# daihangpku/SW-NeRF

Measured on AMD Instinct MI355X. Metric: rays/sec (64+128 samples/ray), higher is better.
Workload: dtype f32

## Files before the change

### __graft_entry__.py

```python
import os
import subprocess
import sys

ROOT = os.path.dirname(os.path.abspath(__file__))
PKG = os.path.join(ROOT, "sw-nerf_amd")
CSRC = os.path.join(PKG, "csrc")
LIB = os.path.join(PKG, "swnerf", "libswnerf_hip.so")
SOURCES = ["render_kernels.hip", "train_kernels.hip", "misc_kernels.hip", "pack_kernels.hip", "backward_kernels.hip", "wgrad_kernels.hip", "wgrad_x3_kernels.hip", "generic_kernels.hip", "x3_kernels.hip", "mesh_kernels.hip", "tnerf_kernels.hip", "tnerf_train_kernels.hip", "metrics_kernels.hip", "pyramid_kernels.hip", "fit2d_kernels.hip", "batch_kernels.hip", "optim_kernels.hip", "patch_kernels.hip", "query_kernels.hip", "image_kernels.hip", "lpips_kernels.hip", "jpeg_kernels.hip", "jpeg_enc_kernels.hip", "marker_kernels.hip", "meshops_kernels.hip", "meshsimp_kernels.hip", "meshfill_kernels.hip"]
HEADERS = ["swnerf_common.h", "mlp_core.h", "mlp_core_x3.h", "bf16x3_split.h", "mlp_kernels.h", "render_pass.h", "composite.h", "resample.h", "wave_dpp.h", "lds_dma.h", "host_util.h", "wgrad_host.h", "mc_tables.h", "elu.h", "ray_rows.h", "tnerf_pass.h", "pyramid_interp.h", "jpeg_math.h", "jpeg_host.h", "jpeg_enc_math.h", "jpeg_enc_host.h", "marker_math.h", "meshops_math.h", "meshops_layout.h", "meshops_common.h", "par_prims.h", "fit2d_cols.h", os.path.join(ROOT, "include", "swnerf.h")]
HIPCC_FLAGS = ["--offload-arch=gfx950", "-O3", "-ffp-contract=off", "-fPIC", "-shared", "-std=c++17"]


OBJDIR = os.path.join(PKG, "build")


def _deps():
    return [os.path.join(CSRC, s) for s in SOURCES] + [h if os.path.isabs(h) else os.path.join(CSRC, h) for h in HEADERS]


def _stale():
    if not os.path.exists(LIB):
        return True
    t = os.path.getmtime(LIB)
    return any(os.path.getmtime(d) > t for d in _deps())


def compile_library(force=False):
    if not (force or _stale()):
        return False
    from concurrent.futures import ThreadPoolExecutor
    hipcc = os.environ.get("HIPCC", "/opt/rocm/bin/hipcc")
# ... 110 lines not shown
```

### include/swnerf.h

```cpp
#ifndef SWNERF_H
#define SWNERF_H
#include <stddef.h>
#include <stdint.h>

#ifdef __cplusplus
extern "C" {
#endif

#define SWNERF_VERSION 112

#define SWNERF_E_ARG      (-1)
#define SWNERF_E_UNSUPP   (-2)
#define SWNERF_E_DATA     (-3)

#define SWNERF_NET_CANON   0
#define SWNERF_NET_DNERF   1
#define SWNERF_NET_NOVIEW  2
#define SWNERF_NET_TNERF   3


int         swnerf_version(void);
const char* swnerf_last_error(void);

size_t swnerf_packed_floats(int kind);
// ... 102 lines not shown
    const float* z_vals;
    int          lindisp;
    const float* t_rand;
    const float* noise;
    int          white_bkgd;
    float* rgb_map;
    float* disp_map;
    float* acc_map;
    float* depth_map;
    float* weights;
    float* raw;
    float* dx;
    float* z_out;
    int          n_importance;
    const float* u;
    float* z_fine;
    float* z_std;
    int          out_ch;
} swnerf_pass_args;

int swnerf_render_pass(const swnerf_pass_args* args , void* stream);

int swnerf_render_pass_ws(const swnerf_pass_args* args , float* view_ws, int64_t view_ws_floats, void* stream);

size_t swnerf_packed_x3_floats_kind(int kind);
int swnerf_pack_net_x3_kind(int kind, const float* const* params , int L_pos, int L_dir, int L_time,
                            const float* packed_fp32, float* packed_x3, void* stream);
size_t swnerf_packed_x3_floats(void);
int swnerf_pack_net_x3(const float* const* params , int L_pos, int L_dir, const float* packed_canon,
                       float* packed_x3, void* stream);
int swnerf_render_pass_x3(const swnerf_pass_args* args , int terms, void* stream);

int64_t swnerf_train_rows(int64_t n_rays, int n_samples);
int swnerf_xs_floats_per_row(void);
int swnerf_render_pass_train(const swnerf_pass_args* args , float* act, float* bits, float* xs, void* stream);
int swnerf_render_pass_backward(const float* packed_bwd, const float* bits, const float* raw ,
                                const float* z_vals , const float* ray_batch, int cols, const float* noise,
                                int64_t n_rays, int n_samples, int white_bkgd, const float* g_rgb ,
                                const float* g_disp , const float* g_acc , const float* g_raw ,
                                float* grad, float* d_raw, void* stream);
size_t swnerf_packed_bwd_noview_floats(void);
int swnerf_pack_net_bwd_noview(const float* const* params , int L_pos, int out_ch,
                               float* packed_bwd, void* stream);
int swnerf_render_pass_backward_noview(const float* packed_bwd, const float* bits, const float* raw ,
                                       const float* z_vals , const float* ray_batch, int cols, const float* noise,
                                       int64_t n_rays, int n_samples, int white_bkgd, int out_ch, const float* g_rgb ,
// ... 210 lines not shown
```

### sw-nerf_amd/csrc/composite.h

```cpp
#pragma once
#include "wave_dpp.h"

typedef float f32x4 __attribute__((ext_vector_type(4)));

__device__ __forceinline__ float comp_dist(bool more, float zn, float z, float dnorm) {
    return (more ? (zn - z) : 1e10f) * dnorm;
}

__device__ __forceinline__ float comp_relu(float sg) { return (sg < 0.f) ? 0.f : sg; }

__device__ __forceinline__ float comp_transmit(float sg, float dist) { return expf(-comp_relu(sg) * dist); }

__device__ __forceinline__ float comp_alpha(float sg, float dist, bool live) {
    return live ? 1.f - comp_transmit(sg, dist) : 0.f;
}

__device__ __forceinline__ double comp_survival(float alpha) { return (double)(1.f - alpha + 1e-10f); }

struct SweepProd { double ex, total; };

template <int W>
__device__ __forceinline__ SweepProd excl_cumprod_shfl(double ps, int l) {
#pragma unroll
    for (int o = 1; o < W; o <<= 1) { const double up = __shfl_up(ps, o, W); if (l >= o) ps *= up; }
// ... 14 lines not shown

__device__ __forceinline__ float comp_sigmoid(float x) { return 1.f / (1.f + expf(-x)); }

__device__ __forceinline__ void comp_accumulate(const float& w, const float& c0, const float& c1, const float& c2, const float& z,
                                                float& pr, float& pg, float& pb, float& pd, float& pa) {
    pr += w * comp_sigmoid(c0);
    pg += w * comp_sigmoid(c1);
    pb += w * comp_sigmoid(c2);
    pd += w * z;
    pa += w;
}

__device__ __forceinline__ void comp_accumulate_density(const float& w, const float& z, float& pd, float& pa) {
    pd += w * z;
    pa += w;
}
__device__ __forceinline__ void comp_accumulate_colour(const float& w, const float& c0, const float& c1, const float& c2,
                                                       float& pr, float& pg, float& pb) {
    pr += w * comp_sigmoid(c0);
    pg += w * comp_sigmoid(c1);
    pb += w * comp_sigmoid(c2);
}

__device__ __forceinline__ void comp_write_maps(float pr, float pg, float pb, float pd, float pa, int white, int64_t ray,
                                                float* rgb_map, float* disp_map, float* acc_map, float* depth_map) {
    if (rgb_map) {
        const float bg = white ? (1.f - pa) : 0.f;
        rgb_map[ray * 3 + 0] = pr + bg;
        rgb_map[ray * 3 + 1] = pg + bg;
        rgb_map[ray * 3 + 2] = pb + bg;
    }
    if (depth_map) depth_map[ray] = pd;
    if (acc_map) acc_map[ray] = pa;
    if (disp_map) {
        const float q = pd / pa;
        disp_map[ray] = 1.f / ((q != q) ? q : fmaxf(1e-10f, q));
    }
}

struct CompGrads { float r, g, b, A, D; bool rgb; };

__device__ __forceinline__ void comp_bwd_fold(CompGrads& g, int white, const float* g_disp, float pd, float pa) {
    if (white) g.A -= (g.r + g.g + g.b);
    if (g_disp) {
        const float q = pd / pa;
        if (q > 1e-10f) { const float gq = -*g_disp / (q * q); g.D += gq / pa; g.A -= gq * pd / (pa * pa); }
    }
}

__device__ __forceinline__ float comp_bwd_G(const CompGrads& g, float c0, float c1, float c2, float z) {
    return (g.rgb ? g.r * c0 + g.g * c1 + g.b * c2 : 0.f) + g.A + g.D * z;
}

__device__ __forceinline__ f32x4 comp_bwd_sample(const CompGrads& g, float G, float T, float w, double R, float sg, float dist,
// ... 9 lines not shown
```

### sw-nerf_amd/csrc/render_kernels.hip

```cpp
#include <hip/hip_runtime.h>
#include "../../include/swnerf.h"
#include "swnerf_common.h"
#include "mlp_core.h"
#include "host_util.h"
#include "mlp_kernels.h"

#include "render_pass.h"

struct QueryDev {
    const float* pts; int64_t M; const float* dirs; int64_t V; int shared;
    const float* w0; const float* b0; int nbias; const float* wvl; float* out;
};

__global__ void __launch_bounds__(256, 1) query_points_kernel(QueryDev P) {
    extern __shared__ __attribute__((aligned(16))) float lds_bias[];
    RowTile rt;
    if (!row_tile(rt, lds_bias, P.b0, P.nbias, P.M)) return;
    f32x16 emb[2], in[8], out[8];
    float head[3];
    pe_pos(P.pts[rt.rr * 3], P.pts[rt.rr * 3 + 1], P.pts[rt.rr * 3 + 2], rt.h, emb);
    WStream ws;
    ws_start(ws, P.w0 + SW_STEPS_DIR * SW_STEP_FLOATS, lds_bias + SW_DIR_BIAS_TILES * SW_BIAS_TILE_FLOATS, rt.lds_ring, rt.lane);
    trunk_pass<false>(emb, rt.lds_emb, 0.f, false, rt.h, in, out, head, ws);
    float rgb[3];
    views_mean(in, ws, P.wvl, P.dirs, P.V, P.shared, rt.rr, rt.h, lds_bias, rgb);
    if (rt.live && rt.h == 0) {
        f32x4 r4 = {rgb[0], rgb[1], rgb[2], head[0]};
        *reinterpret_cast<f32x4*>(P.out + rt.row * 4) = r4;
    }
}

int sw_tnerf_render_launch(const swnerf_pass_args& a, hipStream_t st);

extern "C" int swnerf_render_pass_ws(const swnerf_pass_args* args, float* view_ws, int64_t view_ws_floats, void* stream) {
    static const PassAccepts accepts = {"render_pass", {SW_COLS(11) | SW_COLS(12), SW_COLS(11) | SW_COLS(12), SW_COLS(8), ~0u },
        SWNERF_E_ARG, "%s: ray_batch must have 11 or 12 columns (use_viewdirs) or 8 (SWNERF_NET_NOVIEW), got %d for kind %d", true, 0};
    if (!args) return sw_fail(SWNERF_E_ARG, "render_pass: NULL args");
    const swnerf_pass_args& a = *args;
    if (a.kind < 0 || a.kind > SWNERF_NET_TNERF) return sw_fail(SWNERF_E_ARG, "unknown net kind %d", a.kind);
    int rc = pass_check(accepts, a);
    if (rc) return rc;
    if (a.kind == SWNERF_NET_TNERF) return sw_tnerf_render_launch(a, (hipStream_t)stream);
    const bool noview = a.kind == SWNERF_NET_NOVIEW;
    if (a.kind == SWNERF_NET_DNERF && a.cols != 12) return sw_fail(SWNERF_E_ARG, "render_pass: D-NeRF needs the frame_time column");
    if (noview && a.dx) return sw_fail(SWNERF_E_ARG, "render_pass: a static net has no position_delta output here");
    PassDev P = pass_dev(a);
    rc = noview ? stream_ptrs_noview(a.packed, a.out_ch, &P.w0, &P.b0, &P.nbias, &P.two_pass)
                : stream_ptrs(a.kind, a.packed, a.run_deform, &P.w0, &P.b0, &P.nbias, &P.two_pass);
    if (rc) return rc;
    P.dir_steps = noview ? 0 : SW_STEPS_DIR;
    P.time_steps = (a.kind == SWNERF_NET_DNERF && P.two_pass) ? SW_STEPS_TIME : 0;
    size_t lds = SW_LDS_FIXED_FLOATS * sizeof(float);
    if ((rc = pass_resampling(accepts.name, a, P, lds))) return rc;
    if (view_ws && view_ws_floats < a.n_rays * (int64_t)SW_DEFER_WS_FLOATS)
        return sw_fail(SWNERF_E_ARG, "render_pass: view_ws holds %lld floats, %lld rays need %lld", (long long)view_ws_floats,
                       (long long)a.n_rays, (long long)(a.n_rays * (int64_t)SW_DEFER_WS_FLOATS));
    P.view_ws = (a.kind == SWNERF_NET_CANON && !a.raw && a.n_samples <= SW_DEFER_SMAX) ? view_ws : nullptr;
    if (P.view_ws && a.n_importance <= 0) lds += 4 * SW_DEFER_LDS_FLOATS * sizeof(float);
    if (a.n_rays == 0) return 0;
    if (P.time_steps) {
        P.tb_off = (int)(lds / sizeof(float));
        lds += 4 * SW_TB_LDS_FLOATS * sizeof(float);
    }
    const dim3 grid((unsigned)((a.n_rays + 3) / 4)), block(256);
    hipStream_t st = (hipStream_t)stream;
    pass_startup_args(P, grid.x, noview ? SW_NOVIEW_STEPS : (a.kind == SWNERF_NET_DNERF && P.two_pass ? SW_DEFORM_STEPS + SW_CANON_STEPS : SW_CANON_STEPS));
    if (noview) hipLaunchKernelGGL((render_pass_kernel<false, false, 0, false>), grid, block, lds, st, P);
    else if (a.kind == SWNERF_NET_DNERF) hipLaunchKernelGGL(render_pass_kernel<true>, grid, block, lds, st, P);
    else {
        if (a.dx) {
            rc = sw_check(hipMemsetAsync(a.dx, 0, (size_t)a.n_rays * a.n_samples * 3 * sizeof(float), st), "render_pass dx fill");
            if (rc) return rc;
        }
        hipLaunchKernelGGL(render_pass_kernel<false>, grid, block, lds, st, P);
    }
    return sw_check(hipGetLastError(), "render_pass launch");
}

extern "C" int swnerf_render_pass(const swnerf_pass_args* args, void* stream) { return swnerf_render_pass_ws(args, nullptr, 0, stream); }

__global__ void __launch_bounds__(256) sample_coarse_kernel(swnerf_pass_args a, float* z_out, float* pts) {
    const int64_t idx = (int64_t)blockIdx.x * 256 + threadIdx.x;
    const int S = a.n_samples;
    if (idx >= a.n_rays * S) return;
    const int64_t ray = idx / S;
    const int s = (int)(idx - ray * S);
    const float* rb = a.ray_batch + ray * a.cols;
    const float z = z_sample(a, ray, rb[6], rb[7], s);
    z_out[idx] = z;
    if (pts) {
        pts[idx * 3 + 0] = rb[0] + rb[3] * z;
        pts[idx * 3 + 1] = rb[1] + rb[4] * z;
        pts[idx * 3 + 2] = rb[2] + rb[5] * z;
    }
}

extern "C" int swnerf_sample_coarse(const float* ray_batch, int64_t n_rays, int cols, int n_samples, int lindisp,
                                    const float* t_rand, float* z_vals, float* pts, void* stream) {
    if (n_rays == 0) return 0;
    if (!ray_batch || !z_vals || n_rays < 0 || n_samples < 1 || cols < 8)
        return sw_fail(SWNERF_E_ARG, "sample_coarse: NULL pointer, n_rays %lld, n_samples %d or cols %d < 8", (long long)n_rays, n_samples, cols);
    swnerf_pass_args a = {};
// ... 72 lines not shown
```

### sw-nerf_amd/csrc/render_pass.h

```cpp
#pragma once
#include <cstdlib>
#include "mlp_kernels.h"
#include "mlp_core_x3.h"
#include "resample.h"
#include "composite.h"
#include "ray_rows.h"

#define SW_LDS_SC 256
#define SW_LDS_SORT 1024
#define SW_LDS_WAVE_FLOATS (3 * SW_LDS_SC + SW_LDS_SORT)

#define SW_DEFER_SMAX 240
#define SW_DEFER_LDS_FLOATS (4 * SW_DEFER_SMAX + 64)
#define SW_DEFER_WS_FLOATS (64 * 256)
static_assert(SW_DEFER_LDS_FLOATS <= SW_LDS_SORT, "the deferred colour scratch shares the sort region");

struct PassDev {
    swnerf_pass_args a;
    const float* w0;
    const float* b0;
    int nbias;
    int two_pass;
    int sort_n, sort_s;
    float* act;
    float* bits;
    float* xs;
    float* act_d; float* bits_d; float* xs_d;
    int dir_steps;
    int time_steps;
    int tb_off;
    int warm_steps;
    int warm_blocks;
    int skew_mode;
    int skew_unit;
    float* view_ws;
};

__device__ __forceinline__ float wave32_sum(float v) {
#pragma unroll
    for (int o = 16; o > 0; o >>= 1) v += __shfl_xor(v, o, 32);
    return v;
}

__device__ __forceinline__ float z_linear(const swnerf_pass_args& a, float near, float far, int s) {
    const float t = sw_linspace(0.f, 1.f, a.n_samples, s);
    if (!a.lindisp) return near * (1.f - t) + far * t;
    return 1.f / (1.f / near * (1.f - t) + 1.f / far * t);
}

__device__ __forceinline__ float z_sample(const swnerf_pass_args& a, int64_t ray, float near, float far, int s) {
    const int S = a.n_samples;
    if (a.z_vals) return a.z_vals[ray * S + s];
    const float zs = z_linear(a, near, far, s);
    if (!a.t_rand) return zs;
    const float upper = (s < S - 1) ? .5f * (z_linear(a, near, far, s + 1) + zs) : zs;
    const float lower = (s > 0) ? .5f * (zs + z_linear(a, near, far, s - 1)) : zs;
    return lower + (upper - lower) * a.t_rand[ray * S + s];
}
// ... 185 lines not shown
            tile_park(lds_dir, lane, demb);
        }
        x3_start(xs, reinterpret_cast<const char*>(P.w0), lds_bias, lds_ring, lane, wv);
    } else {
        ws_start(ws, P.w0, lds_bias, lds_ring, lane);
        if constexpr (VIEWS) {
            f32x16 demb;
            pe_dir(v0, v1, v2, h, demb);
            if constexpr (TRAIN) tile_park(lds_dir, lane, demb);
            view_bias_tile(demb, lds_vb, lane, ws);
        }
        if constexpr (DNERF) {
            if (P.time_steps) time_bias_tile(ft, h, lds_all + P.tb_off + wv * SW_TB_LDS_FLOATS, lane, ws);
        }
    }

    const float* zrow = a.z_vals ? a.z_vals + ray * S : nullptr;
    const float* zslot = PREC ? lds_x3w + X3Lds<DNERF>::DIR : lds_emb + SW_EMB_LDS_FLOATS;
    const unsigned zslot_addr = __builtin_amdgcn_readfirstlane((unsigned)(size_t)zslot);
    float pr = 0.f, pg = 0.f, pb = 0.f, pd = 0.f, pa = 0.f;
    double Tc = 1.0;
    const int ntiles = (S + 31) >> 5;
    constexpr bool DEFER_OK = !DNERF && !TRAIN && PREC == 0 && VIEWS;
    const bool defer = DEFER_OK && P.view_ws != nullptr;
    float* dW = resample ? srt : lds_all + PassLds<DNERF, TRAIN>::FIXED + wv * SW_DEFER_LDS_FLOATS;
    float* dC = dW + SW_DEFER_SMAX;
    int* dIdx = reinterpret_cast<int*>(dW + 4 * SW_DEFER_SMAX);
    float* vrow = DEFER_OK ? P.view_ws + ray * SW_DEFER_WS_FLOATS + h * 128 : nullptr;
    const char* main_head = reinterpret_cast<const char*>(P.w0 + (P.dir_steps + P.time_steps) * SW_STEP_FLOATS);
    const char* viewsh_head = main_head + (SW_CANON_MAIN_STEPS - SW_STEPS_VIEWSH) * 1024;
    int pend = 0, wr = 0, rd = 0;
    if constexpr (DEFER_OK) {
        if (defer) {
            for (int i = lane; i < 3 * SW_DEFER_SMAX; i += 64) dC[i] = 0.f;
            wave_lds_sync();
        }
    }
#pragma nounroll
    for (int tile = 0; tile < ntiles || (DEFER_OK && pend > 0); ++tile) {
        const bool is_tile = !DEFER_OK || tile < ntiles;
        const bool flush = !defer || !is_tile || pend >= 32;
        const int s = tile * 32 + j;
        const bool live = s < S && !ghost;
        const int sc = live ? s : S - 1;
        float z, zn;
        if (zrow && tile > 0) {
            const float* zs = zslot + (tile & 1) * 64;
            z = zs[j];
            const float z1 = zs[j + 1];
            zn = (s + 1 < S) ? z1 : z;
        } else {
            z = z_sample(a, ray, near, far, sc);
            zn = (s + 1 < S) ? z_sample(a, ray, near, far, s + 1) : z;
        }
        if (zrow && tile + 1 < ntiles)
            lds_dma_dword(reinterpret_cast<const char*>(zrow), (unsigned)min(32 * (tile + 1) + lane, S - 1) * 4u,
                          zslot_addr + (unsigned)((tile + 1) & 1) * 256u);
        float px = ox + dx * z, py = oy + dy * z, pz = oz + dz * z;

        f32x16 emb[2], in[8], out[8];
        float head[3], rgb[3];
        float extra = 0.f;
        if (is_tile) pe_pos(px, py, pz, h, emb);
        if (DNERF && TRAIN) {
            const int64_t tix = ray * ntiles + tile, prow = tix * 32 + j;
            float* act_row = P.act + prow * SW_ACT_LD + 4 * h;
            float* mask_tile = P.bits + tix * SW_MASK_TILE_FLOATS + lane * 4;
            float* xs_row = P.xs + prow * SW_XS_LD + 4 * h;
            f32x4 mb = {0.f, 0.f, 0.f, 0.f};
            f32x16 demb;
#pragma nounroll
            for (int pass = 0; pass < 2; ++pass) {
                const bool dp = pass == 0;
                trunk_pass<true, true, true, false, true>(emb, lds_emb, ft, dp, h, in, out, head, ws,
                                             dp ? P.act_d + prow * SW_ACT_LD + 4 * h : act_row,
                                             dp ? P.bits_d + tix * SW_MASK_TILE_FLOATS + lane * 4 : mask_tile, dp, &mb,
                                             dp ? P.xs_d + prow * SW_XS_LD + 4 * h : xs_row, lds_tb);
                if (dp) {
                    const float ex = head[0], ey = head[1], ez = head[2];
                    if (live && h == 0) {
                        float* o = a.dx + (ray * S + s) * 3;
                        o[0] = ex; o[1] = ey; o[2] = ez;
                    }
                    px = px + ex; py = py + ey; pz = pz + ez;
                    pe_pos(px, py, pz, h, emb);
                    tile_fetch(lds_dir, lane, demb);
// ... 63 lines not shown
            f32x4 mb = {0.f, 0.f, 0.f, 0.f};
            f32x16 demb;
            tile_fetch(lds_dir, lane, demb);
#pragma unroll
            for (int g = 0; g < 4; ++g) {
                const f32x4 v = {demb[4 * g], demb[4 * g + 1], demb[4 * g + 2], demb[4 * g + 3]};
                *reinterpret_cast<f32x4*>(xs_row + 64 + 8 * g) = v;
            }
            trunk_pass<false, true, true>(emb, lds_emb, 0.f, false, h, in, out, head, ws, act_row, mask_tile, false, &mb, xs_row);
            canon_tail_train(in, lds_vb, rgb, ws.bias - SW_BIAS_TILE_FLOATS, ws, act_row, mask_tile, mb);
        } else if constexpr (PREC != 0) {
            head[1] = 0.f; head[2] = 0.f;
            x3_canon_pipe<PREC>(px, py, pz, h, lds_dir, lane, head[0], rgb, xs);
            x3_rewind(xs, SW_X3_CANON_CHUNKS, lds_bias, lane);
        } else if constexpr (!VIEWS) {
            trunk_pass<false, false, false, true>(emb, lds_emb, 0.f, false, h, in, out, head, ws);
            float o5[5] = {0.f, 0.f, 0.f, 0.f, 0.f};
            const int nout = (a.out_ch == 5 && !a.raw) ? 4 : a.out_ch;
            head_valu_rt<8>(in, ws, nout, o5);
            ws.bias += (a.out_ch - nout) * 8 * SW_BIAS_TILE_FLOATS;
            rgb[0] = o5[0] + ws.bias[0]; rgb[1] = o5[1] + ws.bias[1]; rgb[2] = o5[2] + ws.bias[2];
            head[0] = o5[3] + ws.bias[3]; head[1] = 0.f; head[2] = 0.f;
            extra = o5[4] + ws.bias[4];
        } else if (is_tile) {
            trunk_pass<false, false, false, false, false, true>(emb, lds_emb, 0.f, false, h, in, out, head, ws, nullptr, nullptr, false,
                                                                nullptr, nullptr, nullptr, (flush || tile + 1 >= ntiles) ? nullptr : main_head);
        }

        const float sg_raw = is_tile ? head[0] : 0.f;
        float sg = sg_raw;
        if (a.noise) sg += a.noise[ray * S + sc];
        const float alpha = comp_alpha(sg, comp_dist(s + 1 < S, zn, z, dnorm), live && is_tile);
        float w = 0.f;
        if (is_tile) {
            w = alpha * comp_transmittance(excl_cumprod_shfl<32>(comp_survival(alpha), j), Tc);
            if (live) {
                if (a.weights && h == 0) a.weights[ray * S + s] = w;
                if (a.z_out && h == 0) a.z_out[ray * S + s] = z;
                if (resample && h == 0) { zc[s] = z; wc[s] = w; }
            }
            comp_accumulate_density(w, z, pd, pa);
        }

        int src_s = s;
        bool src_ok = live;
        if constexpr (DEFER_OK) {
            if (defer) {
                const bool lit = is_tile && live && (!(alpha == 0.f) || s == 0);
                const unsigned m = (unsigned)__ballot(lit);
                const unsigned below = (1u << j) - 1u;
                const int cnt = __builtin_amdgcn_readfirstlane(__popc(m));
                if (live && is_tile && h == 0) dW[s] = w;
                if (!flush) {
                    const int slot = (wr + __popc(m & below)) & 63;
                    if (lit) {
                        if (h == 0) dIdx[slot] = s;
                        float* q = vrow + slot * 256;
#pragma unroll
                        for (int c = 0; c < 32; ++c) {
                            const f32x4 v = {in[c >> 2][4 * (c & 3)], in[c >> 2][4 * (c & 3) + 1], in[c >> 2][4 * (c & 3) + 2], in[c >> 2][4 * (c & 3) + 3]};
                            *reinterpret_cast<f32x4*>(q + c * 4) = v;
                        }
                    }
                    wr += cnt; pend += cnt;
                } else {
                    const int room = 32 - cnt, nv = pend < room ? pend : room;
                    const int rank = __popc(~m & below);
                    src_ok = lit || rank < nv;
                    if (!lit && (rank < nv || !is_tile)) {
                        const int slot = (rd + (rank < nv ? rank : nv - 1)) & 63;
                        src_s = dIdx[slot];
                        const float* p = vrow + slot * 256;
#pragma unroll
                        for (int c = 0; c < 32; ++c) {
                            const f32x4 v = *reinterpret_cast<const f32x4*>(p + c * 4);
                            in[c >> 2][4 * (c & 3) + 0] = v[0]; in[c >> 2][4 * (c & 3) + 1] = v[1];
                            in[c >> 2][4 * (c & 3) + 2] = v[2]; in[c >> 2][4 * (c & 3) + 3] = v[3];
                        }
                    }
                    rd += nv; pend -= nv;
                    if (!is_tile) ws.bias = lds_bias + (SW_DIR_BIAS_TILES + 64 + 8 + 1) * SW_BIAS_TILE_FLOATS + h * 16;
                }
                wave_lds_sync();
            }
        }
        const bool drain_next = DEFER_OK && tile + 1 >= ntiles && pend > 0;
        if (!TRAIN && PREC == 0 && VIEWS) {
            if (flush) {
                if constexpr (DEFER_OK) ws.cont = drain_next ? viewsh_head : ws.base + SW_STEPS_VIEWSH * 1024;
                canon_tail<DEFER_OK>(in, lds_vb, rgb, ws.bias - SW_BIAS_TILE_FLOATS, ws);
            }
        }
        if constexpr (PREC == 0) {
            ws_rewind(ws, P.w0 + (P.dir_steps + P.time_steps) * SW_STEP_FLOATS,
                      lds_bias + ((P.dir_steps ? SW_DIR_BIAS_TILES : 0) + (P.time_steps ? 8 : 0)) * SW_BIAS_TILE_FLOATS, lane);
            if (drain_next) ws.base = viewsh_head;
        }

        const float c0 = rgb[0], c1 = rgb[1], c2 = rgb[2];
        if (DEFER_OK && defer) {
            if (flush && src_ok && h == 0) { dC[src_s] = c0; dC[SW_DEFER_SMAX + src_s] = c1; dC[2 * SW_DEFER_SMAX + src_s] = c2; }
            continue;
        }
        if (a.raw && live && h == 0) {
            if (!VIEWS && a.out_ch == 5) {
                float* o = a.raw + (ray * S + s) * 5;
                o[0] = c0; o[1] = c1; o[2] = c2; o[3] = sg_raw; o[4] = extra;
            } else {
                f32x4 r4 = {c0, c1, c2, sg_raw};
                *reinterpret_cast<f32x4*>(a.raw + (ray * S + s) * 4) = r4;
            }
        }
        comp_accumulate_colour(w, c0, c1, c2, pr, pg, pb);
    }

    if constexpr (DEFER_OK) {
        if (defer) {
            wave_lds_sync();
#pragma nounroll
            for (int t = 0; t < ntiles; ++t) {
                const int s = t * 32 + j;
                const int sc = s < S ? s : S - 1;
                const float w = s < S ? dW[sc] : 0.f;
                const float c0 = dC[sc], c1 = dC[SW_DEFER_SMAX + sc], c2 = dC[2 * SW_DEFER_SMAX + sc];
                comp_accumulate_colour(w, c0, c1, c2, pr, pg, pb);
            }
        }
    }
    pr = wave32_sum(pr); pg = wave32_sum(pg); pb = wave32_sum(pb);
    pd = wave32_sum(pd); pa = wave32_sum(pa);
    if (lane == 0 && !ghost) comp_write_maps(pr, pg, pb, pd, pa, a.white_bkgd, ray, a.rgb_map, a.disp_map, a.acc_map, a.depth_map);
    if (!resample || ghost) return;

    wave_lds_sync();
    const int Ni = a.n_importance;
    const double sm = wave_sample_pdf(wc + 1, S - 1, MidBins{zc}, a.u ? a.u + ray * Ni : nullptr, Ni, cdf, srt, lane);
    if (a.z_std) {
        const float sd = wave_zstd(sm, srt, Ni, lane);
        if (lane == 0) a.z_std[ray] = sd;
    }
    wave_rank_merge(zc, S, P.sort_s, srt, Ni, P.sort_n, a.z_fine + ray * (S + Ni), lane);
}
```

### sw-nerf_amd/swnerf/render.py

```python
import inspect
import os

import numpy as np
import torch

from . import _lib
from .ray import get_rays, sample_pdf, raw2outputs
from .embedder import EmbedFn, to8b
from .png import write_png
from .model import vallina_NeRF, NeRFOriginal, DirectTemporalNeRF

DEBUG = False
PASS_HOOK = None
Z_TAP = None


def batchify(fn, chunk):
    if chunk is None:
        return fn

    def ret(inputs):
        return torch.cat([fn(inputs[i:i + chunk]) for i in range(0, inputs.shape[0], chunk)], 0)
    return ret

# ... 101 lines not shown
    N, cols = rb.shape
    Ni = int(n_importance)
    a = _lib.PassArgs()
    a.ray_batch, a.n_rays, a.cols, a.kind, a.packed = rb.data_ptr(), N, cols, kind, packed.data_ptr()
    a.run_deform, (a.L_pos, a.L_dir, a.L_time), a.n_samples, a.out_ch = int(bool(run_deform)), bands, S, out_ch
    a.lindisp, a.white_bkgd, a.n_importance = int(bool(lindisp)), int(bool(white_bkgd)), Ni
    keep = [rb, packed]
    for name, t in inputs.items():
        if t is not None:
            t = _lib.dev_f32(t, name, Ni if name == "u" else S)
            if t.shape[0] != N:
                raise ValueError(f"swnerf.{who}: {name} must have {N} rows, got {tuple(t.shape)}")
            keep.append(t)
            setattr(a, name, t.data_ptr())
    shapes = {"rgb_map": (N, 3), "disp_map": (N,), "acc_map": (N,), "depth_map": (N,), "weights": (N, S), "raw": (N, S, out_ch),
              "dx": (N, S, 3), "z_out": (N, S), "z_fine": (N, S + Ni), "z_std": (N,)}
    out = {k: torch.empty(shapes[k], dtype=torch.float32, device=rb.device) for k in list(outputs) + (["z_fine", "z_std"] if Ni > 0 else [])}
    for k, t in out.items():
        setattr(a, k, t.data_ptr())
    return a, out, keep


VIEW_WS_FLOATS_PER_RAY = 64 * 256
VIEW_WS_SMAX = 240
_VIEW_WS = {}


def view_workspace(rb, n_rays):
    key = (rb.device, torch.cuda.current_stream(rb.device).cuda_stream)
    ws = _VIEW_WS.get(key)
    if ws is None or ws.numel() < n_rays * VIEW_WS_FLOATS_PER_RAY:
        _VIEW_WS[key] = ws = torch.empty(n_rays * VIEW_WS_FLOATS_PER_RAY, dtype=torch.float32, device=rb.device)
    return ws


def render_pass(ray_batch, net, n_samples, *, z_vals=None, lindisp=False, t_rand=None, noise=None, white_bkgd=False,
                want=("rgb_map", "disp_map", "acc_map"), n_importance=0, u=None, run_deform=True, precision=None):
    noview = isinstance(net, vallina_NeRF) and net._noview_params() is not None
    out_ch = 4
    if noview:
        packed, Lp, out_ch = net.packed_noview()
        kind, Ld, Lt, terms = _lib.NET_NOVIEW, 0, 0, 0
        if _PRECISIONS[PRECISION if precision is None else precision] and not _WARNED.get("noview_x3"):
            _WARNED["noview_x3"] = True
            import warnings
            warnings.warn(f"swnerf: precision {PRECISION if precision is None else precision!r} was requested, but the bf16 paths are built for the "
                          "nets WITH view directions only - this use_viewdirs=False net renders in fp32 (label your numbers accordingly)")
    else:
        kind, packed, Lp, Ld, Lt = net.packed()
        mode = PRECISION if precision is None else precision
        terms = _PRECISIONS[mode]
        if mode == "bf16x3-fine" and n_importance > 0:
            terms = 0
        if terms:
            packed, _, _ = net.packed_x3()
    rb = _lib.dev_f32(ray_batch, "ray_batch")
    N, S = rb.shape[0], int(n_samples)
    a, out, _keep = pass_args(rb, kind, packed, (Lp, Ld, Lt), S, out_ch, run_deform, dict(z_vals=z_vals, t_rand=t_rand, noise=noise, u=u),
                              want, n_importance, lindisp=lindisp, white_bkgd=white_bkgd)
    if PASS_HOOK is not None:
        PASS_HOOK("begin", N, S)
    if terms:
        _lib.check(_lib.lib().swnerf_render_pass_x3(a, terms, _lib.stream_of(rb)), "render_pass_x3")
    else:
        if kind == _lib.NET_CANON and "raw" not in want and S <= VIEW_WS_SMAX and N > 0:
            ws = view_workspace(rb, N)
            _lib.check(_lib.lib().swnerf_render_pass_ws(a, _lib.ptr(ws), ws.numel(), _lib.stream_of(rb)), "render_pass")
        else:
            _lib.check(_lib.lib().swnerf_render_pass(a, _lib.stream_of(rb)), "render_pass")
    if PASS_HOOK is not None:
        PASS_HOOK("end", N, S)
    return out


def chunked_backward(rb, act_rows, div, widths, launch, gemm_jobs, rest_on_main=True):
    from .wgrad import _Fan, _chunk_gemms
    N = rb.shape[0]
    rows_per_ray = act_rows // N
    chunk = max(4, (TRAIN_BWD_CHUNK_ROWS // div // rows_per_ray) // 4 * 4)
    bufs = [torch.empty((min(N, chunk) * rows_per_ray, w), dtype=torch.float32, device=rb.device) for w in widths]
    fan = _Fan(rb.device)
    for r0 in range(0, N, chunk):
        r1 = min(N, r0 + chunk)
        launch(r0, r1, bufs)
        _chunk_gemms(_lib.lib(), fan, (r1 - r0) * rows_per_ray, gemm_jobs(r0 * rows_per_ray, r1 * rows_per_ray, (r1 - r0) * rows_per_ray, bufs),
                     rest_on_main=rest_on_main)


def f32_grads(*gs):
# ... 363 lines not shown
```

Baseline: 551,800.

## Split deferred view-colour head into global compaction and separate dense kernels

Replaces the in-kernel, per-wave LDS ring that deferred the view-dependent colour head for non-empty samples. Now the main pass stashes trunk features of lit samples into a global workspace. A prefix-scan kernel compacts them across all rays, a dense colour kernel runs the view head over 32-row segments, and a final kernel composites rgb. The aim is to remove the per-ray padding and drain waste of evaluating the colour head on partly empty tiles. The cost is much more global memory traffic (257 floats per stashed row, up to an 8 GB workspace), a single-block scan, and two extra launches.

After: 560,400, median of 6. 1.02x the previous value.

```diff
diff --git a/__graft_entry__.py b/__graft_entry__.py
--- a/__graft_entry__.py
+++ b/__graft_entry__.py
@@ -6,7 +6,7 @@
 PKG = os.path.join(ROOT, "sw-nerf_amd")
 CSRC = os.path.join(PKG, "csrc")
 LIB = os.path.join(PKG, "swnerf", "libswnerf_hip.so")
-SOURCES = ["render_kernels.hip", "train_kernels.hip", "misc_kernels.hip", "pack_kernels.hip", "backward_kernels.hip", "wgrad_kernels.hip", "wgrad_x3_kernels.hip", "generic_kernels.hip", "x3_kernels.hip", "mesh_kernels.hip", "tnerf_kernels.hip", "tnerf_train_kernels.hip", "metrics_kernels.hip", "pyramid_kernels.hip", "fit2d_kernels.hip", "batch_kernels.hip", "optim_kernels.hip", "patch_kernels.hip", "query_kernels.hip", "image_kernels.hip", "lpips_kernels.hip", "jpeg_kernels.hip", "jpeg_enc_kernels.hip", "marker_kernels.hip", "meshops_kernels.hip", "meshsimp_kernels.hip", "meshfill_kernels.hip"]
+SOURCES = ["render_kernels.hip", "colour_kernels.hip", "train_kernels.hip", "misc_kernels.hip", "pack_kernels.hip", "backward_kernels.hip", "wgrad_kernels.hip", "wgrad_x3_kernels.hip", "generic_kernels.hip", "x3_kernels.hip", "mesh_kernels.hip", "tnerf_kernels.hip", "tnerf_train_kernels.hip", "metrics_kernels.hip", "pyramid_kernels.hip", "fit2d_kernels.hip", "batch_kernels.hip", "optim_kernels.hip", "patch_kernels.hip", "query_kernels.hip", "image_kernels.hip", "lpips_kernels.hip", "jpeg_kernels.hip", "jpeg_enc_kernels.hip", "marker_kernels.hip", "meshops_kernels.hip", "meshsimp_kernels.hip", "meshfill_kernels.hip"]
 HEADERS = ["swnerf_common.h", "mlp_core.h", "mlp_core_x3.h", "bf16x3_split.h", "mlp_kernels.h", "render_pass.h", "composite.h", "resample.h", "wave_dpp.h", "lds_dma.h", "host_util.h", "wgrad_host.h", "mc_tables.h", "elu.h", "ray_rows.h", "tnerf_pass.h", "pyramid_interp.h", "jpeg_math.h", "jpeg_host.h", "jpeg_enc_math.h", "jpeg_enc_host.h", "marker_math.h", "meshops_math.h", "meshops_layout.h", "meshops_common.h", "par_prims.h", "fit2d_cols.h", os.path.join(ROOT, "include", "swnerf.h")]
 HIPCC_FLAGS = ["--offload-arch=gfx950", "-O3", "-ffp-contract=off", "-fPIC", "-shared", "-std=c++17"]
 
diff --git a/include/swnerf.h b/include/swnerf.h
--- a/include/swnerf.h
+++ b/include/swnerf.h
@@ -148,6 +148,7 @@
 int swnerf_render_pass(const swnerf_pass_args* args , void* stream);
 
 int swnerf_render_pass_ws(const swnerf_pass_args* args , float* view_ws, int64_t view_ws_floats, void* stream);
+int64_t swnerf_view_ws_floats(int64_t n_rays, int n_samples);
 
 size_t swnerf_packed_x3_floats_kind(int kind);
 int swnerf_pack_net_x3_kind(int kind, const float* const* params , int L_pos, int L_dir, int L_time,
diff --git a/sw-nerf_amd/csrc/colour_kernels.hip b/sw-nerf_amd/csrc/colour_kernels.hip
--- /dev/null
+++ b/sw-nerf_amd/csrc/colour_kernels.hip
@@ -0,0 +1,128 @@
+#include <hip/hip_runtime.h>
+#include "../../include/swnerf.h"
+#include "swnerf_common.h"
+#include "mlp_core.h"
+#include "host_util.h"
+#include "mlp_kernels.h"
+#include "render_pass.h"
+
+__global__ void __launch_bounds__(1024) colour_scan_kernel(ViewWs vw, int64_t n_rays) {
+    __shared__ int part[16];
+    const int tid = threadIdx.x, lane = tid & 63, wv = tid >> 6;
+    const int64_t K = (n_rays + 1023) / 1024;
+    const int64_t r0 = tid * K, r1 = r0 + K < n_rays ? r0 + K : n_rays;
+    int* off = vw_off(vw);
+    int* segray = vw_segray(vw, n_rays);
+    int sum = 0;
+    for (int64_t r = r0; r < r1; ++r) sum += off[r];
+    int v = sum;
+#pragma unroll
+    for (int o = 1; o < 64; o <<= 1) { const int up = __shfl_up(v, o, 64); if (lane >= o) v += up; }
+    if (lane == 63) part[wv] = v;
+    __syncthreads();
+    int below = v - sum, total = 0;
+#pragma unroll
+    for (int k = 0; k < 16; ++k) { if (k < wv) below += part[k]; total += part[k]; }
+    for (int64_t r = r0; r < r1; ++r) {
+        const int cnt = off[r];
+        off[r] = below;
+        for (int g = (below + 31) >> 5; 32 * g < below + cnt; ++g) segray[g] = (int)r;
+        below += cnt;
+    }
+    if (tid == 0) off[n_rays] = total;
+}
+
+struct ColourDev {
+    ViewWs vw;
+    const float* ray_batch; int cols; int64_t n_rays;
+    const float* b0; int nbias;
+    const float* wvl;
+};
+
+__global__ void __launch_bounds__(256, 2) colour_rows_kernel(ColourDev P) {
+    extern __shared__ __attribute__((aligned(16))) float lds_bias[];
+    const int lane = threadIdx.x & 63, j = lane & 31, h = lane >> 5;
+    const int wv = __builtin_amdgcn_readfirstlane(threadIdx.x >> 6);
+    bias_to_lds(lds_bias, P.b0, P.nbias);
+    const int* off = vw_off(P.vw);
+    const int* segray = vw_segray(P.vw, P.n_rays);
+    const int total = __builtin_amdgcn_readfirstlane(off[P.n_rays]);
+    const int nseg = (total + 31) >> 5, nwaves = (int)gridDim.x * 4;
+    int g = (int)blockIdx.x * 4 + wv;
+    if (g >= nseg) return;
+    WStream ws;
+    ws_start(ws, P.wvl, lds_bias, lds_bias + P.nbias + wv * SW_RING * SW_STEP_FLOATS, lane);
+    const float* rgb_tiles = ws.bias + (SW_DIR_BIAS_TILES + 64 + 8 + 1) * SW_BIAS_TILE_FLOATS;
+    const float* hb_rgb = rgb_tiles - SW_BIAS_TILE_FLOATS;
+    const int gs = vw_group_stride(P.vw);
+#pragma nounroll
+    for (; g < nseg; g += nwaves) {
+        const int row = 32 * g + j;
+        const bool valid = row < total;
+        const int i = valid ? row : total - 1;
+        const int rg = __builtin_amdgcn_readfirstlane(segray[g]);
+        const int64_t rk = (int64_t)rg + j + 1;
+        const int nxt = off[rk < P.n_rays ? rk : P.n_rays];
+        int dr = 0;
+#pragma unroll
+        for (int k = 0; k < 32; ++k) dr += (__shfl(nxt, k, 32) <= i) ? 1 : 0;
+        const int64_t ray = (int64_t)rg + dr;
+        const int slot = i - off[ray];
+        float* reg = vw_ray(P.vw, ray);
+        const int s = vw_sample(P.vw, reg)[slot];
+        const float* q = vw_row(P.vw, reg, slot, h);
+        f32x16 in[8], demb, hv[4];
+#pragma unroll
+        for (int c = 0; c < 32; ++c) {
+            const f32x4 v = *reinterpret_cast<const f32x4*>(q + (size_t)c * gs);
+            in[c >> 2][4 * (c & 3) + 0] = v[0]; in[c >> 2][4 * (c & 3) + 1] = v[1];
+            in[c >> 2][4 * (c & 3) + 2] = v[2]; in[c >> 2][4 * (c & 3) + 3] = v[3];
+        }
+        const float* dp = P.ray_batch + ray * P.cols + (P.cols - 3);
+        pe_dir(dp[0], dp[1], dp[2], h, demb);
+        ws.bias = rgb_tiles;
+        ws.base = reinterpret_cast<const char*>(P.wvl);
+        canon_tail_rows(in, demb, hv, lds_bias + h * 16, ws);
+        float c3[3];
+        head_valu<3, 4>(hv, ws, c3);
+        if (valid && h == 0) {
+            float* c = vw_c(P.vw, reg);
+            c[s] = c3[0] + hb_rgb[1]; c[P.vw.sp + s] = c3[1] + hb_rgb[2]; c[2 * P.vw.sp + s] = c3[2] + hb_rgb[3];
+        }
+    }
+}
+
+__global__ void __launch_bounds__(256) colour_maps_kernel(ViewWs vw, int64_t n_rays, int S, int white, float* rgb_map) {
+    const int lane = threadIdx.x & 63, j = lane & 31;
+    const int64_t ray = (int64_t)blockIdx.x * 4 + (threadIdx.x >> 6);
+    if (ray >= n_rays) return;
+    float* reg = vw_ray(vw, ray);
+    const float* wq = vw_w(vw, reg);
+    const float* cq = vw_c(vw, reg);
+    float pr = 0.f, pg = 0.f, pb = 0.f;
+    const int ntiles = (S + 31) >> 5;
+#pragma nounroll
+    for (int t = 0; t < ntiles; ++t) {
+        const int s = t * 32 + j;
+        const int sc = s < S ? s : S - 1;
+        const float w = s < S ? wq[sc] : 0.f;
+        const float c0 = cq[sc], c1 = cq[vw.sp + sc], c2 = cq[2 * vw.sp + sc];
+        comp_accumulate_colour(w, c0, c1, c2, pr, pg, pb);
+    }
+    pr = wave32_sum(pr); pg = wave32_sum(pg); pb = wave32_sum(pb);
+    if (lane == 0) comp_write_rgb(pr, pg, pb, reg[0], white, ray, rgb_map);
+}
+
+int sw_colour_split_launch(const swnerf_pass_args& a, const ViewWs& vw, const float* b0, int nbias, const float* wvl, hipStream_t st) {
+    hipLaunchKernelGGL(colour_scan_kernel, dim3(1), dim3(1024), 0, st, vw, a.n_rays);
+    const int64_t rows_max = a.n_rays * (int64_t)(vw.rows < a.n_samples ? vw.rows : a.n_samples);
+    const int64_t wgs = (rows_max + 127) / 128;
+    if (wgs > 0) {
+        ColourDev P;
+        P.vw = vw; P.ray_batch = a.ray_batch; P.cols = a.cols; P.n_rays = a.n_rays; P.b0 = b0; P.nbias = nbias; P.wvl = wvl;
+        const size_t lds = ((size_t)nbias + 4 * SW_RING * SW_STEP_FLOATS) * sizeof(float);
+        hipLaunchKernelGGL(colour_rows_kernel, dim3((unsigned)(wgs < 512 ? wgs : 512)), dim3(256), lds, st, P);
+    }
+    hipLaunchKernelGGL(colour_maps_kernel, dim3((unsigned)((a.n_rays + 3) / 4)), dim3(256), 0, st, vw, a.n_rays, a.n_samples, a.white_bkgd, a.rgb_map);
+    return sw_check(hipGetLastError(), "render_pass colour launch");
+}
diff --git a/sw-nerf_amd/csrc/composite.h b/sw-nerf_amd/csrc/composite.h
--- a/sw-nerf_amd/csrc/composite.h
+++ b/sw-nerf_amd/csrc/composite.h
@@ -60,14 +60,16 @@
     pb += w * comp_sigmoid(c2);
 }
 
+__device__ __forceinline__ void comp_write_rgb(float pr, float pg, float pb, float pa, int white, int64_t ray, float* rgb_map) {
+    const float bg = white ? (1.f - pa) : 0.f;
+    rgb_map[ray * 3 + 0] = pr + bg;
+    rgb_map[ray * 3 + 1] = pg + bg;
+    rgb_map[ray * 3 + 2] = pb + bg;
+}
+
 __device__ __forceinline__ void comp_write_maps(float pr, float pg, float pb, float pd, float pa, int white, int64_t ray,
                                                 float* rgb_map, float* disp_map, float* acc_map, float* depth_map) {
-    if (rgb_map) {
-        const float bg = white ? (1.f - pa) : 0.f;
-        rgb_map[ray * 3 + 0] = pr + bg;
-        rgb_map[ray * 3 + 1] = pg + bg;
-        rgb_map[ray * 3 + 2] = pb + bg;
-    }
+    if (rgb_map) comp_write_rgb(pr, pg, pb, pa, white, ray, rgb_map);
     if (depth_map) depth_map[ray] = pd;
     if (acc_map) acc_map[ray] = pa;
     if (disp_map) {
diff --git a/sw-nerf_amd/csrc/render_kernels.hip b/sw-nerf_amd/csrc/render_kernels.hip
--- a/sw-nerf_amd/csrc/render_kernels.hip
+++ b/sw-nerf_amd/csrc/render_kernels.hip
@@ -31,6 +31,7 @@
 }
 
 int sw_tnerf_render_launch(const swnerf_pass_args& a, hipStream_t st);
+int sw_colour_split_launch(const swnerf_pass_args& a, const ViewWs& vw, const float* b0, int nbias, const float* wvl, hipStream_t st);
 
 extern "C" int swnerf_render_pass_ws(const swnerf_pass_args* args, float* view_ws, int64_t view_ws_floats, void* stream) {
     static const PassAccepts accepts = {"render_pass", {SW_COLS(11) | SW_COLS(12), SW_COLS(11) | SW_COLS(12), SW_COLS(8), ~0u },
@@ -55,8 +56,7 @@
     if (view_ws && view_ws_floats < a.n_rays * (int64_t)SW_DEFER_WS_FLOATS)
         return sw_fail(SWNERF_E_ARG, "render_pass: view_ws holds %lld floats, %lld rays need %lld", (long long)view_ws_floats,
                        (long long)a.n_rays, (long long)(a.n_rays * (int64_t)SW_DEFER_WS_FLOATS));
-    P.view_ws = (a.kind == SWNERF_NET_CANON && !a.raw && a.n_samples <= SW_DEFER_SMAX) ? view_ws : nullptr;
-    if (P.view_ws && a.n_importance <= 0) lds += 4 * SW_DEFER_LDS_FLOATS * sizeof(float);
+    if (view_ws && a.kind == SWNERF_NET_CANON && !a.raw && a.n_samples <= SW_DEFER_SMAX) P.vw = view_ws_layout(view_ws, view_ws_floats, a.n_rays, a.n_samples);
     if (a.n_rays == 0) return 0;
     if (P.time_steps) {
         P.tb_off = (int)(lds / sizeof(float));
@@ -73,11 +73,21 @@
             if (rc) return rc;
         }
         hipLaunchKernelGGL(render_pass_kernel<false>, grid, block, lds, st, P);
+        if (P.vw.base && a.rgb_map) {
+            if ((rc = sw_check(hipGetLastError(), "render_pass launch"))) return rc;
+            return sw_colour_split_launch(a, P.vw, P.b0, P.nbias, views_loop_ptr(a.kind, a.packed), st);
+        }
     }
     return sw_check(hipGetLastError(), "render_pass launch");
 }
 
 extern "C" int swnerf_render_pass(const swnerf_pass_args* args, void* stream) { return swnerf_render_pass_ws(args, nullptr, 0, stream); }
+
+extern "C" int64_t swnerf_view_ws_floats(int64_t n_rays, int n_samples) {
+    if (n_rays <= 0 || n_samples <= 0) return 0;
+    const int64_t full = view_ws_full(n_rays, n_samples), least = n_rays * (int64_t)SW_DEFER_WS_FLOATS;
+    return full > least ? full : least;
+}
 
 __global__ void __launch_bounds__(256) sample_coarse_kernel(swnerf_pass_args a, float* z_out, float* pts) {
     const int64_t idx = (int64_t)blockIdx.x * 256 + threadIdx.x;
diff --git a/sw-nerf_amd/csrc/render_pass.h b/sw-nerf_amd/csrc/render_pass.h
--- a/sw-nerf_amd/csrc/render_pass.h
+++ b/sw-nerf_amd/csrc/render_pass.h
@@ -11,9 +11,40 @@
 #define SW_LDS_WAVE_FLOATS (3 * SW_LDS_SC + SW_LDS_SORT)
 
 #define SW_DEFER_SMAX 240
-#define SW_DEFER_LDS_FLOATS (4 * SW_DEFER_SMAX + 64)
 #define SW_DEFER_WS_FLOATS (64 * 256)
-static_assert(SW_DEFER_LDS_FLOATS <= SW_LDS_SORT, "the deferred colour scratch shares the sort region");
+#define SW_DEFER_SEGS_PER_RAY ((SW_DEFER_SMAX + 31) / 32)
+
+struct ViewWs {
+    float* base;
+    int64_t hdr, per_ray;
+    int rows, sp;
+};
+
+static inline int64_t view_ws_hdr(int64_t n_rays) { return ((n_rays + 1 + 3) & ~(int64_t)3) + SW_DEFER_SEGS_PER_RAY * n_rays; }
+static inline int64_t view_ws_full(int64_t n_rays, int S) {
+    const int64_t sp = (S + 3) & ~3;
+    return view_ws_hdr(n_rays) + n_rays * (4 + 4 * sp + 257 * sp);
+}
+static inline ViewWs view_ws_layout(float* base, int64_t floats, int64_t n_rays, int S) {
+    ViewWs v = {};
+    v.base = base;
+    v.sp = (S + 3) & ~3;
+    v.hdr = view_ws_hdr(n_rays);
+    const int64_t avail = n_rays > 0 ? ((floats - v.hdr) / n_rays) & ~(int64_t)3 : 0;
+    int64_t r = ((avail - 4 - 4 * v.sp) / 257) & ~(int64_t)3;
+    if (r > v.sp) r = v.sp;
+    v.rows = r > 0 ? (int)r : 0;
+    v.per_ray = 4 + 4 * (int64_t)v.sp + 257 * (int64_t)v.rows;
+    return v;
+}
+__device__ __forceinline__ int* vw_off(const ViewWs& v) { return reinterpret_cast<int*>(v.base); }
+__device__ __forceinline__ int* vw_segray(const ViewWs& v, int64_t n_rays) { return reinterpret_cast<int*>(v.base) + ((n_rays + 1 + 3) & ~(int64_t)3); }
+__device__ __forceinline__ float* vw_ray(const ViewWs& v, int64_t ray) { return v.base + v.hdr + ray * v.per_ray; }
+__device__ __forceinline__ float* vw_w(const ViewWs& v, float* reg) { return reg + 4; }
+__device__ __forceinline__ float* vw_c(const ViewWs& v, float* reg) { return reg + 4 + v.sp; }
+__device__ __forceinline__ int* vw_sample(const ViewWs& v, float* reg) { return reinterpret_cast<int*>(reg + 4 + 4 * v.sp); }
+__device__ __forceinline__ float* vw_row(const ViewWs& v, float* reg, int slot, int h) { return reg + 4 + 4 * v.sp + v.rows + (h * v.rows + slot) * 4; }
+__device__ __forceinline__ int vw_group_stride(const ViewWs& v) { return 8 * v.rows; }
 
 struct PassDev {
     swnerf_pass_args a;
@@ -33,7 +64,7 @@
     int warm_blocks;
     int skew_mode;
     int skew_unit;
-    float* view_ws;
+    ViewWs vw;
 };
 
 __device__ __forceinline__ float wave32_sum(float v) {
@@ -265,24 +296,13 @@
     double Tc = 1.0;
     const int ntiles = (S + 31) >> 5;
     constexpr bool DEFER_OK = !DNERF && !TRAIN && PREC == 0 && VIEWS;
-    const bool defer = DEFER_OK && P.view_ws != nullptr;
-    float* dW = resample ? srt : lds_all + PassLds<DNERF, TRAIN>::FIXED + wv * SW_DEFER_LDS_FLOATS;
-    float* dC = dW + SW_DEFER_SMAX;
-    int* dIdx = reinterpret_cast<int*>(dW + 4 * SW_DEFER_SMAX);
-    float* vrow = DEFER_OK ? P.view_ws + ray * SW_DEFER_WS_FLOATS + h * 128 : nullptr;
+    const bool defer = DEFER_OK && P.vw.base != nullptr;
+    float* vreg = defer ? vw_ray(P.vw, ray) : nullptr;
     const char* main_head = reinterpret_cast<const char*>(P.w0 + (P.dir_steps + P.time_steps) * SW_STEP_FLOATS);
-    const char* viewsh_head = main_head + (SW_CANON_MAIN_STEPS - SW_STEPS_VIEWSH) * 1024;
-    int pend = 0, wr = 0, rd = 0;
-    if constexpr (DEFER_OK) {
-        if (defer) {
-            for (int i = lane; i < 3 * SW_DEFER_SMAX; i += 64) dC[i] = 0.f;
-            wave_lds_sync();
-        }
-    }
+    int wr = 0;
 #pragma nounroll
-    for (int tile = 0; tile < ntiles || (DEFER_OK && pend > 0); ++tile) {
-        const bool is_tile = !DEFER_OK || tile < ntiles;
-        const bool flush = !defer || !is_tile || pend >= 32;
+    for (int tile = 0; tile < ntiles; ++tile) {
+        const bool stash = defer && wr + min(32, S - tile * 32) <= P.vw.rows;
         const int s = tile * 32 + j;
         const bool live = s < S && !ghost;
         const int sc = live ? s : S - 1;
@@ -304,7 +324,7 @@
         f32x16 emb[2], in[8], out[8];
         float head[3], rgb[3];
         float extra = 0.f;
-        if (is_tile) pe_pos(px, py, pz, h, emb);
+        pe_pos(px, py, pz, h, emb);
         if (DNERF && TRAIN) {
             const int64_t tix = ray * ntiles + tile, prow = tix * 32 + j;
             float* act_row = P.act + prow * SW_ACT_LD + 4 * h;
@@ -414,84 +434,65 @@
             rgb[0] = o5[0] + ws.bias[0]; rgb[1] = o5[1] + ws.bias[1]; rgb[2] = o5[2] + ws.bias[2];
             head[0] = o5[3] + ws.bias[3]; head[1] = 0.f; head[2] = 0.f;
             extra = o5[4] + ws.bias[4];
-        } else if (is_tile) {
+        } else {
             trunk_pass<false, false, false, false, false, true>(emb, lds_emb, 0.f, false, h, in, out, head, ws, nullptr, nullptr, false,
-                                                                nullptr, nullptr, nullptr, (flush || tile + 1 >= ntiles) ? nullptr : main_head);
-        }
-
-        const float sg_raw = is_tile ? head[0] : 0.f;
+                                                                nullptr, nullptr, nullptr, stash ? main_head : nullptr);
+        }
+
+        const float sg_raw = head[0];
         float sg = sg_raw;
         if (a.noise) sg += a.noise[ray * S + sc];
-        const float alpha = comp_alpha(sg, comp_dist(s + 1 < S, zn, z, dnorm), live && is_tile);
-        float w = 0.f;
-        if (is_tile) {
-            w = alpha * comp_transmittance(excl_cumprod_shfl<32>(comp_survival(alpha), j), Tc);
-            if (live) {
-                if (a.weights && h == 0) a.weights[ray * S + s] = w;
-                if (a.z_out && h == 0) a.z_out[ray * S + s] = z;
-                if (resample && h == 0) { zc[s] = z; wc[s] = w; }
-            }
-            comp_accumulate_density(w, z, pd, pa);
-        }
-
-        int src_s = s;
-        bool src_ok = live;
+        const float alpha = comp_alpha(sg, comp_dist(s + 1 < S, zn, z, dnorm), live);
+        const float w = alpha * comp_transmittance(excl_cumprod_shfl<32>(comp_survival(alpha), j), Tc);
+        if (live) {
+            if (a.weights && h == 0) a.weights[ray * S + s] = w;
+            if (a.z_out && h == 0) a.z_out[ray * S + s] = z;
+            if (resample && h == 0) { zc[s] = z; wc[s] = w; }
+        }
+        comp_accumulate_density(w, z, pd, pa);
+
+        bool lit = live;
         if constexpr (DEFER_OK) {
             if (defer) {
-                const bool lit = is_tile && live && (!(alpha == 0.f) || s == 0);
-                const unsigned m = (unsigned)__ballot(lit);
-                const unsigned below = (1u << j) - 1u;
-                const int cnt = __builtin_amdgcn_readfirstlane(__popc(m));
-                if (live && is_tile && h == 0) dW[s] = w;
-                if (!flush) {
-                    const int slot = (wr + __popc(m & below)) & 63;
+                lit = live && (!(alpha == 0.f) || s == 0);
+                if (live && h == 0) vw_w(P.vw, vreg)[s] = w;
+                if (stash) {
+                    const unsigned m = (unsigned)__ballot(lit);
+                    const int slot = wr + __popc(m & ((1u << j) - 1u));
                     if (lit) {
-                        if (h == 0) dIdx[slot] = s;
-                        float* q = vrow + slot * 256;
+                        if (h == 0) vw_sample(P.vw, vreg)[slot] = s;
+                        float* q = vw_row(P.vw, vreg, slot, h);
+                        const int gs = vw_group_stride(P.vw);
 #pragma unroll
                         for (int c = 0; c < 32; ++c) {
                             const f32x4 v = {in[c >> 2][4 * (c & 3)], in[c >> 2][4 * (c & 3) + 1], in[c >> 2][4 * (c & 3) + 2], in[c >> 2][4 * (c & 3) + 3]};
-                            *reinterpret_cast<f32x4*>(q + c * 4) = v;
+                            *reinterpret_cast<f32x4*>(q + (size_t)c * gs) = v;
                         }
                     }
-                    wr += cnt; pend += cnt;
-                } else {
-                    const int room = 32 - cnt, nv = pend < room ? pend : room;
-                    const int rank = __popc(~m & below);
-                    src_ok = lit || rank < nv;
-                    if (!lit && (rank < nv || !is_tile)) {
-                        const int slot = (rd + (rank < nv ? rank : nv - 1)) & 63;
-                        src_s = dIdx[slot];
-                        const float* p = vrow + slot * 256;
-#pragma unroll
-                        for (int c = 0; c < 32; ++c) {
-                            const f32x4 v = *reinterpret_cast<const f32x4*>(p + c * 4);
-                            in[c >> 2][4 * (c & 3) + 0] = v[0]; in[c >> 2][4 * (c & 3) + 1] = v[1];
-                            in[c >> 2][4 * (c & 3) + 2] = v[2]; in[c >> 2][4 * (c & 3) + 3] = v[3];
-                        }
-                    }
-                    rd += nv; pend -= nv;
-                    if (!is_tile) ws.bias = lds_bias + (SW_DIR_BIAS_TILES + 64 + 8 + 1) * SW_BIAS_TILE_FLOATS + h * 16;
+                    wr += __builtin_amdgcn_readfirstlane(__popc(m));
                 }
-                wave_lds_sync();
-            }
-        }
-        const bool drain_next = DEFER_OK && tile + 1 >= ntiles && pend > 0;
+            }
+        }
         if (!TRAIN && PREC == 0 && VIEWS) {
-            if (flush) {
-                if constexpr (DEFER_OK) ws.cont = drain_next ? viewsh_head : ws.base + SW_STEPS_VIEWSH * 1024;
+            if (!stash) {
+                if constexpr (DEFER_OK) ws.cont = ws.base + SW_STEPS_VIEWSH * 1024;
                 canon_tail<DEFER_OK>(in, lds_vb, rgb, ws.bias - SW_BIAS_TILE_FLOATS, ws);
+            } else {
+                rgb[0] = 0.f; rgb[1] = 0.f; rgb[2] = 0.f;
             }
         }
         if constexpr (PREC == 0) {
             ws_rewind(ws, P.w0 + (P.dir_steps + P.time_steps) * SW_STEP_FLOATS,
                       lds_bias + ((P.dir_steps ? SW_DIR_BIAS_TILES : 0) + (P.time_steps ? 8 : 0)) * SW_BIAS_TILE_FLOATS, lane);
-            if (drain_next) ws.base = viewsh_head;
         }
 
         const float c0 = rgb[0], c1 = rgb[1], c2 = rgb[2];
         if (DEFER_OK && defer) {
-            if (flush && src_ok && h == 0) { dC[src_s] = c0; dC[SW_DEFER_SMAX + src_s] = c1; dC[2 * SW_DEFER_SMAX + src_s] = c2; }
+            if (live && h == 0) {
+                float* c = vw_c(P.vw, vreg);
+                const bool here = lit && !stash;
+                c[s] = here ? c0 : 0.f; c[P.vw.sp + s] = here ? c1 : 0.f; c[2 * P.vw.sp + s] = here ? c2 : 0.f;
+            }
             continue;
         }
         if (a.raw && live && h == 0) {
@@ -506,22 +507,12 @@
         comp_accumulate_colour(w, c0, c1, c2, pr, pg, pb);
     }
 
-    if constexpr (DEFER_OK) {
-        if (defer) {
-            wave_lds_sync();
-#pragma nounroll
-            for (int t = 0; t < ntiles; ++t) {
-                const int s = t * 32 + j;
-                const int sc = s < S ? s : S - 1;
-                const float w = s < S ? dW[sc] : 0.f;
-                const float c0 = dC[sc], c1 = dC[SW_DEFER_SMAX + sc], c2 = dC[2 * SW_DEFER_SMAX + sc];
-                comp_accumulate_colour(w, c0, c1, c2, pr, pg, pb);
-            }
-        }
-    }
     pr = wave32_sum(pr); pg = wave32_sum(pg); pb = wave32_sum(pb);
     pd = wave32_sum(pd); pa = wave32_sum(pa);
-    if (lane == 0 && !ghost) comp_write_maps(pr, pg, pb, pd, pa, a.white_bkgd, ray, a.rgb_map, a.disp_map, a.acc_map, a.depth_map);
+    if (lane == 0 && !ghost) comp_write_maps(pr, pg, pb, pd, pa, a.white_bkgd, ray, defer ? nullptr : a.rgb_map, a.disp_map, a.acc_map, a.depth_map);
+    if constexpr (DEFER_OK) {
+        if (defer && lane == 0) { vw_off(P.vw)[ray] = wr; vreg[0] = pa; }
+    }
     if (!resample || ghost) return;
 
     wave_lds_sync();
diff --git a/sw-nerf_amd/swnerf/render.py b/sw-nerf_amd/swnerf/render.py
--- a/sw-nerf_amd/swnerf/render.py
+++ b/sw-nerf_amd/swnerf/render.py
@@ -147,15 +147,18 @@
 
 
 VIEW_WS_FLOATS_PER_RAY = 64 * 256
+VIEW_WS_BUDGET_BYTES = 8 << 30
 VIEW_WS_SMAX = 240
 _VIEW_WS = {}
 
 
-def view_workspace(rb, n_rays):
+def view_workspace(rb, n_rays, n_samples):
+    full = int(_lib.lib().swnerf_view_ws_floats(n_rays, n_samples))
+    floats = max(n_rays * VIEW_WS_FLOATS_PER_RAY, min(full, VIEW_WS_BUDGET_BYTES // 4))
     key = (rb.device, torch.cuda.current_stream(rb.device).cuda_stream)
     ws = _VIEW_WS.get(key)
-    if ws is None or ws.numel() < n_rays * VIEW_WS_FLOATS_PER_RAY:
-        _VIEW_WS[key] = ws = torch.empty(n_rays * VIEW_WS_FLOATS_PER_RAY, dtype=torch.float32, device=rb.device)
+    if ws is None or ws.numel() < floats:
+        _VIEW_WS[key] = ws = torch.empty(floats, dtype=torch.float32, device=rb.device)
     return ws
 
 
@@ -189,7 +192,7 @@
         _lib.check(_lib.lib().swnerf_render_pass_x3(a, terms, _lib.stream_of(rb)), "render_pass_x3")
     else:
         if kind == _lib.NET_CANON and "raw" not in want and S <= VIEW_WS_SMAX and N > 0:
-            ws = view_workspace(rb, N)
+            ws = view_workspace(rb, N, S)
             _lib.check(_lib.lib().swnerf_render_pass_ws(a, _lib.ptr(ws), ws.numel(), _lib.stream_of(rb)), "render_pass")
         else:
             _lib.check(_lib.lib().swnerf_render_pass(a, _lib.stream_of(rb)), "render_pass")
```
